# jannerm/ddpo

Hardware: AMD Instinct MI355X
Metric: sampled images/sec (512^2, 50 DDIM steps) (higher is better)
Workload: dtype f32 (f16mx: f16 MFMA + MX-fp8 cross terms on the long-reduction conv/GEMM layers, bf16x3-split MFMA elsewhere); 1 GPU; BASELINE configs[1]: compressed-animals geometry, sd15 U-Net+VAE (random init), 512x512, 50 DDIM steps, CFG 5.0, eta 1.0, sample_batch_size 8/GPU, VAE decode included; parallelism=dp1, global_batch=8

## Files before the change

ddpo_amd/csrc/attention_bf16.hip:

```cpp
#include "common.h"
#include <cstdlib>


typedef __bf16 bf16x8 __attribute__((ext_vector_type(8)));
typedef _Float16 f16x8 __attribute__((ext_vector_type(8)));
typedef _Float16 f16x2 __attribute__((ext_vector_type(2)));
typedef float f32x16 __attribute__((ext_vector_type(16)));

typedef __bf16 bf16x2 __attribute__((ext_vector_type(2)));
__device__ __forceinline__ uint32_t cvt_pk_bf16_a(float lo, float hi) {
  const bf16x2 v = {(__bf16)lo, (__bf16)hi};
  return __builtin_bit_cast(uint32_t, v);
}
__device__ __forceinline__ uint32_t cvt_pk_f16_a(float lo, float hi) {
  const f16x2 v = {(_Float16)lo, (_Float16)hi};
  return __builtin_bit_cast(uint32_t, v);
}
__device__ __forceinline__ void split2(float a, float b, uint32_t& hi, uint32_t& lo) {
  hi = cvt_pk_bf16_a(a, b);
  lo = cvt_pk_bf16_a(a - __uint_as_float(hi << 16), b - __uint_as_float(hi & 0xFFFF0000u));
}
__device__ __forceinline__ void split2h(float a, float b, uint32_t& hi, uint32_t& lo) {
  const float lim = 65504.f;
  a = fminf(fmaxf(a, -lim), lim);
  b = fminf(fmaxf(b, -lim), lim);
  hi = cvt_pk_f16_a(a, b);
  const f16x2 h = __builtin_bit_cast(f16x2, hi);
  lo = cvt_pk_f16_a(a - (float)h[0], b - (float)h[1]);
}
#define MFMA32(a, b, c) __builtin_amdgcn_mfma_f32_32x32x16_bf16((a), (b), (c), 0, 0, 0)
#define MFMA32H(a, b, c) __builtin_amdgcn_mfma_f32_32x32x16_f16((a), (b), (c), 0, 0, 0)
#define ATTN_P_SHIFT 14.0f
#define ATTN_F16_ONE 0x3C00u

template <bool ONES>
__device__ __forceinline__ void attn_softmax_tile(const f32x16 (&sacc)[2], float& m_run, float& l_run, f16x8 (&ph)[4], float& alpha, bool& grew) {
  float mx = sacc[0][0];
#pragma unroll
  for (int j = 0; j < 2; ++j)
#pragma unroll
    for (int r = 0; r < 16; ++r) mx = fmaxf(mx, sacc[j][r]);
  mx = fmaxf(mx, __shfl_xor(mx, 32, 64));
  const float m_new = fmaxf(m_run, mx);
  alpha = __builtin_amdgcn_exp2f(m_run - m_new);
  grew = m_new > m_run;
  m_run = m_new;
  const float m_sh = m_new - ATTN_P_SHIFT;
  float ls = 0.f;
#pragma unroll
  for (int j = 0; j < 2; ++j) {
#pragma unroll
    for (int half = 0; half < 2; ++half) {
      uint32_t pk[4];
#pragma unroll
      for (int e = 0; e < 4; ++e) {
        const float p0 = __builtin_amdgcn_exp2f(sacc[j][8 * half + 2 * e] - m_sh);
        const float p1 = __builtin_amdgcn_exp2f(sacc[j][8 * half + 2 * e + 1] - m_sh);
        pk[e] = cvt_pk_f16_a(p0, p1);
        if (!ONES) {
          const f16x2 q = __builtin_bit_cast(f16x2, pk[e]);
          ls += (float)q[0] + (float)q[1];
        }
      }
      ph[2 * j + half] = __builtin_bit_cast(f16x8, make_uint4(pk[0], pk[1], pk[2], pk[3]));
    }
  }
  if (!ONES) l_run = l_run * alpha + ls;
}

template <int NDT, int LDVT, int QB = 1>
__device__ __forceinline__ void attn_pv_tile(const char* Vhi, const char* Vlo, int li, int h, const f16x8 (*ph)[4], f32x16 (*oacc)[NDT]) {
  f16x8 vh[2][NDT], vl[2][NDT];
  auto fetch = [&](int u, int slot) {
#pragma unroll
    for (int n = 0; n < NDT; ++n) {
      const int off = ((32 * n + li) * LDVT + 16 * u + 4 * h) * 2;
      const uint2 a0 = *reinterpret_cast<const uint2*>(Vhi + off), a1 = *reinterpret_cast<const uint2*>(Vhi + off + 16);
      const uint2 c0 = *reinterpret_cast<const uint2*>(Vlo + off), c1 = *reinterpret_cast<const uint2*>(Vlo + off + 16);
      vh[slot][n] = __builtin_bit_cast(f16x8, make_uint4(a0.x, a0.y, a1.x, a1.y));
      vl[slot][n] = __builtin_bit_cast(f16x8, make_uint4(c0.x, c0.y, c1.x, c1.y));
    }
  };
  fetch(0, 0);
#pragma unroll
  for (int u = 0; u < 4; ++u) {
    if (u + 1 < 4) fetch(u + 1, (u + 1) & 1);
    __builtin_amdgcn_sched_barrier(0);
#pragma unroll
    for (int qb = 0; qb < QB; ++qb)
#pragma unroll
      for (int n = 0; n < NDT; ++n) oacc[qb][n] = MFMA32H(vl[u & 1][n], ph[qb][u], oacc[qb][n]);
#pragma unroll
    for (int qb = 0; qb < QB; ++qb)
#pragma unroll
      for (int n = 0; n < NDT; ++n) oacc[qb][n] = MFMA32H(vh[u & 1][n], ph[qb][u], oacc[qb][n]);
    __builtin_amdgcn_sched_barrier(0);
  }
}

template <int D, int NDT, bool ONES>
__device__ __forceinline__ float attn_row_sum(const f32x16 (&oacc)[NDT], float l_run, int li) {
  if constexpr (ONES) {
    constexpr int n1 = D / 32, r1 = D % 32;
    static_assert(r1 % 8 == 0 && n1 < NDT, "row D must be register 4 (r1 / 8) of the lanes with h == 0");
    return __shfl(oacc[n1][4 * (r1 / 8)], li, 64);
  } else {
    return l_run + __shfl_xor(l_run, 32, 64);
  }
}

__device__ __forceinline__ void attn_softmax_tile_x3(const f32x16 (&sacc)[2], float& m_run, float& l_run, bf16x8 (&ph)[4], bf16x8 (&pl)[4], float& alpha,
                                                     bool& grew) {
  float mx = sacc[0][0];
#pragma unroll
  for (int j = 0; j < 2; ++j)
#pragma unroll
    for (int r = 0; r < 16; ++r) mx = fmaxf(mx, sacc[j][r]);
  mx = fmaxf(mx, __shfl_xor(mx, 32, 64));
  const float m_new = fmaxf(m_run, mx);
  alpha = __builtin_amdgcn_exp2f(m_run - m_new);
  grew = m_new > m_run;
  m_run = m_new;
  float ls = 0.f;
#pragma unroll
  for (int j = 0; j < 2; ++j) {
#pragma unroll
    for (int half = 0; half < 2; ++half) {
      uint32_t hi[4], lo[4];
#pragma unroll
      for (int e = 0; e < 4; ++e) {
        const float p0 = __builtin_amdgcn_exp2f(sacc[j][8 * half + 2 * e] - m_new);
        const float p1 = __builtin_amdgcn_exp2f(sacc[j][8 * half + 2 * e + 1] - m_new);
        ls += p0 + p1;
        split2(p0, p1, hi[e], lo[e]);
      }
      ph[2 * j + half] = __builtin_bit_cast(bf16x8, make_uint4(hi[0], hi[1], hi[2], hi[3]));
      pl[2 * j + half] = __builtin_bit_cast(bf16x8, make_uint4(lo[0], lo[1], lo[2], lo[3]));
    }
  }
  l_run = l_run * alpha + ls;
}

template <int NDT, int LDVT, int QB = 1>
__device__ __forceinline__ void attn_pv_tile_x3(const char* Vhi, const char* Vlo, int li, int h, const bf16x8 (*ph)[4], const bf16x8 (*pl)[4],
                                                f32x16 (*oacc)[NDT]) {
#pragma unroll
  for (int u = 0; u < 4; ++u) {
#pragma unroll
    for (int n = 0; n < NDT; ++n) {
      const int off = ((32 * n + li) * LDVT + 16 * u + 4 * h) * 2;
      const uint2 a0 = *reinterpret_cast<const uint2*>(Vhi + off), a1 = *reinterpret_cast<const uint2*>(Vhi + off + 16);
      const uint2 c0 = *reinterpret_cast<const uint2*>(Vlo + off), c1 = *reinterpret_cast<const uint2*>(Vlo + off + 16);
      const bf16x8 vh = __builtin_bit_cast(bf16x8, make_uint4(a0.x, a0.y, a1.x, a1.y));
      const bf16x8 vl = __builtin_bit_cast(bf16x8, make_uint4(c0.x, c0.y, c1.x, c1.y));
#pragma unroll
      for (int qb = 0; qb < QB; ++qb) {
        oacc[qb][n] = MFMA32(vl, ph[qb][u], oacc[qb][n]);
        oacc[qb][n] = MFMA32(vh, pl[qb][u], oacc[qb][n]);
        oacc[qb][n] = MFMA32(vh, ph[qb][u], oacc[qb][n]);
      }
    }
  }
}

template <bool F16P, bool ONES, int NDT, int LDVT>
__device__ __forceinline__ void attn_tile_tail(const f32x16 (&sacc)[2], float& m_run, float& l_run, f32x16 (&oacc)[NDT], const char* Vhi, const char* Vlo,
                                               int li, int h) {
  float alpha;
  bool grew;
  if constexpr (F16P) {
    f16x8 ph[4];
    attn_softmax_tile<ONES>(sacc, m_run, l_run, ph, alpha, grew);
    if (__any(grew)) {
#pragma unroll
      for (int n = 0; n < NDT; ++n)
#pragma unroll
        for (int r = 0; r < 16; ++r) oacc[n][r] *= alpha;
    }
    attn_pv_tile<NDT, LDVT>(Vhi, Vlo, li, h, &ph, &oacc);
  } else {
    bf16x8 ph[4], pl[4];
    attn_softmax_tile_x3(sacc, m_run, l_run, ph, pl, alpha, grew);
    if (__any(grew)) {
#pragma unroll
      for (int n = 0; n < NDT; ++n)
#pragma unroll
        for (int r = 0; r < 16; ++r) oacc[n][r] *= alpha;
    }
    attn_pv_tile_x3<NDT, LDVT>(Vhi, Vlo, li, h, &ph, &pl, &oacc);
  }
}

struct AttnOut {
  float* o;
  uint16_t* hi;
  uint16_t* lo;
  int ld;
  int64_t rows;
};
template <int D, int NDT>
__device__ __forceinline__ void attn_store_o(const AttnOut out, int64_t row, int col0, const f32x16 (&oacc)[NDT], float inv, int h) {
#pragma unroll
  for (int n = 0; n < NDT; ++n) {
#pragma unroll
    for (int g = 0; g < 4; ++g) {
      const int dc = 32 * n + 8 * g + 4 * h;
      if (dc >= D) continue;
      const float v0 = oacc[n][4 * g] * inv, v1 = oacc[n][4 * g + 1] * inv, v2 = oacc[n][4 * g + 2] * inv, v3 = oacc[n][4 * g + 3] * inv;
      if (out.hi) {
        uint32_t h0, l0, h1, l1;
        split2(v0, v1, h0, l0);
        split2(v2, v3, h1, l1);
        const int64_t off = plane_off(row, col0 + dc, out.ld, out.rows);
        *reinterpret_cast<uint2*>(out.hi + off) = make_uint2(h0, h1);
        *reinterpret_cast<uint2*>(out.lo + off) = make_uint2(l0, l1);
      } else {
        *reinterpret_cast<float4*>(out.o + row * out.ld + col0 + dc) = make_float4(v0, v1, v2, v3);
      }
    }
  }
}


template <int D, int DKP, int DVP, bool F16P>
__global__ void __launch_bounds__(256) attn_fwd_bf16_kernel(const float* __restrict__ q, int ldq, const float* __restrict__ k, int ldk,
                                                            const float* __restrict__ v, int ldv, const AttnOut out,
                                                            float* __restrict__ lse, int heads, int Nq, int Nk, float scale_log2e, int qbat) {
  constexpr int KT = 64;
  constexpr int LDK = DKP + 8;
  constexpr int LDVT = KT + 4;
  constexpr int NKS = DKP / 16;
  constexpr int NDT = DVP / 32;
  constexpr bool ONES = F16P && DVP > D;
  constexpr int K_BYTES = KT * LDK * 2, VT_BYTES = DVP * LDVT * 2;
  __shared__ __attribute__((aligned(16))) char smem[2 * K_BYTES + 2 * VT_BYTES];
  char* Khi = smem; char* Klo = smem + K_BYTES;
  char* Vhi = smem + 2 * K_BYTES; char* Vlo = Vhi + VT_BYTES;

  const int t = threadIdx.x, lane = t & 63, wid = t >> 6;
  const int li = lane & 31, h = lane >> 5;
  const int bh = blockIdx.y, b = bh / heads, hd = bh - b * heads;
  const int q0 = blockIdx.x * 128 + wid * 32;
  const int qrow = min(q0 + li, Nq - 1);

  bf16x8 qh[NKS], ql[NKS];
  {
    const float* qp = q + ((int64_t)(b % qbat) * Nq + qrow) * ldq + hd * D;
#pragma unroll
    for (int s = 0; s < NKS; ++s) {
      uint32_t hi[4], lo[4];
#pragma unroll
      for (int e = 0; e < 4; ++e) {
        const int dk = 16 * s + 8 * h + 2 * e;
        const float a = dk < D ? qp[dk] * scale_log2e : 0.f;
        const float c = dk + 1 < D ? qp[dk + 1] * scale_log2e : 0.f;
        split2(a, c, hi[e], lo[e]);
      }
      qh[s] = __builtin_bit_cast(bf16x8, make_uint4(hi[0], hi[1], hi[2], hi[3]));
      ql[s] = __builtin_bit_cast(bf16x8, make_uint4(lo[0], lo[1], lo[2], lo[3]));
    }
  }
  for (int i = t; i < (2 * K_BYTES + 2 * VT_BYTES) / 16; i += 256) reinterpret_cast<uint4*>(smem)[i] = make_uint4(0u, 0u, 0u, 0u);
  if constexpr (ONES) {
    __syncthreads();
    if (t < KT) reinterpret_cast<uint16_t*>(Vhi)[D * LDVT + t] = (uint16_t)ATTN_F16_ONE;
  }

  f32x16 oacc[NDT];
#pragma unroll
  for (int n = 0; n < NDT; ++n)
#pragma unroll
    for (int r = 0; r < 16; ++r) oacc[n][r] = 0.f;
  float m_run = -INFINITY, l_run = 0.f;
  const float* kb = k + (int64_t)b * Nk * ldk + hd * D;
  const float* vb = v + (int64_t)b * Nk * ldv + hd * D;

  for (int kt0 = 0; kt0 < Nk; kt0 += KT) {
    __syncthreads();
    for (int i = t; i < KT * (D / 4); i += 256) {
      const int key = i / (D / 4), c4 = i - key * (D / 4);
      float4 kv = make_float4(0.f, 0.f, 0.f, 0.f), vv = kv;
      if (kt0 + key < Nk) {
        kv = *reinterpret_cast<const float4*>(kb + (int64_t)(kt0 + key) * ldk + c4 * 4);
        vv = *reinterpret_cast<const float4*>(vb + (int64_t)(kt0 + key) * ldv + c4 * 4);
      }
      uint32_t h0, l0, h1, l1;
      split2(kv.x, kv.y, h0, l0);
      split2(kv.z, kv.w, h1, l1);
      *reinterpret_cast<uint2*>(Khi + (key * LDK + c4 * 4) * 2) = make_uint2(h0, h1);
      *reinterpret_cast<uint2*>(Klo + (key * LDK + c4 * 4) * 2) = make_uint2(l0, l1);
      if (F16P) { split2h(vv.x, vv.y, h0, l0); split2h(vv.z, vv.w, h1, l1); }
      else { split2(vv.x, vv.y, h0, l0); split2(vv.z, vv.w, h1, l1); }
      uint16_t* vh = reinterpret_cast<uint16_t*>(Vhi);
      uint16_t* vl = reinterpret_cast<uint16_t*>(Vlo);
      const int d0 = c4 * 4;
      vh[(d0 + 0) * LDVT + key] = (uint16_t)(h0 & 0xFFFFu); vh[(d0 + 1) * LDVT + key] = (uint16_t)(h0 >> 16);
      vh[(d0 + 2) * LDVT + key] = (uint16_t)(h1 & 0xFFFFu); vh[(d0 + 3) * LDVT + key] = (uint16_t)(h1 >> 16);
      vl[(d0 + 0) * LDVT + key] = (uint16_t)(l0 & 0xFFFFu); vl[(d0 + 1) * LDVT + key] = (uint16_t)(l0 >> 16);
      vl[(d0 + 2) * LDVT + key] = (uint16_t)(l1 & 0xFFFFu); vl[(d0 + 3) * LDVT + key] = (uint16_t)(l1 >> 16);
    }
    __syncthreads();

    f32x16 sacc[2];
#pragma unroll
    for (int j = 0; j < 2; ++j)
#pragma unroll
      for (int r = 0; r < 16; ++r) sacc[j][r] = 0.f;
#pragma unroll
    for (int s = 0; s < NKS; ++s) {
#pragma unroll
      for (int j = 0; j < 2; ++j) {
        const int off = ((j * 32 + li) * LDK + 16 * s + 8 * h) * 2;
        const bf16x8 kh = *reinterpret_cast<const bf16x8*>(Khi + off);
        const bf16x8 kl = *reinterpret_cast<const bf16x8*>(Klo + off);
        sacc[j] = MFMA32(kl, qh[s], sacc[j]);
        sacc[j] = MFMA32(kh, ql[s], sacc[j]);
        sacc[j] = MFMA32(kh, qh[s], sacc[j]);
      }
    }
    if (kt0 + KT > Nk) {
#pragma unroll
      for (int j = 0; j < 2; ++j)
#pragma unroll
        for (int r = 0; r < 16; ++r)
          if (kt0 + 32 * j + (r & 3) + 8 * (r >> 2) + 4 * h >= Nk) sacc[j][r] = -INFINITY;
    }
    attn_tile_tail<F16P, ONES, NDT, LDVT>(sacc, m_run, l_run, oacc, Vhi, Vlo, li, h);
  }

  const float l_tot = attn_row_sum<D, NDT, ONES>(oacc, l_run, li);
  const float inv = 1.0f / l_tot;
  if (lse && h == 0 && q0 + li < Nq) lse[(int64_t)bh * Nq + q0 + li] = m_run + log2f(l_tot) - (F16P ? ATTN_P_SHIFT : 0.f);
  if (q0 + li < Nq) attn_store_o<D, NDT>(out, (int64_t)b * Nq + q0 + li, hd * D, oacc, inv, h);
}

template <int D, int DKP, int DVP>
struct AttnImg {
  static constexpr int KT = 64, LDK = DKP + 8, LDVT = KT + 4;
  static constexpr int K_BYTES = KT * LDK * 2, VT_BYTES = DVP * LDVT * 2;
  static constexpr int BYTES = 2 * K_BYTES + 2 * VT_BYTES;
  static constexpr int CHUNKS = BYTES / 16;
};

template <int D, int DKP, int DVP, bool F16P>
__global__ void __launch_bounds__(256) attn_pack_kv_kernel(const float* __restrict__ k, int ldk, const float* __restrict__ v, int ldv,
                                                           uint4* __restrict__ img, int heads, int Nk, int ntiles) {
  using I = AttnImg<D, DKP, DVP>;
  __shared__ __attribute__((aligned(16))) char smem[I::BYTES];
  char* Khi = smem; char* Klo = smem + I::K_BYTES;
  char* Vhi = smem + 2 * I::K_BYTES; char* Vlo = Vhi + I::VT_BYTES;
  const int t = threadIdx.x;
  const int tile = blockIdx.x, bh = blockIdx.y, b = bh / heads, hd = bh - b * heads;
  const int kt0 = tile * I::KT;
  for (int i = t; i < I::CHUNKS; i += 256) reinterpret_cast<uint4*>(smem)[i] = make_uint4(0u, 0u, 0u, 0u);
  __syncthreads();
  if (F16P && DVP > D && t < I::KT) reinterpret_cast<uint16_t*>(Vhi)[D * I::LDVT + t] = (uint16_t)ATTN_F16_ONE;
  const float* kb = k + (int64_t)b * Nk * ldk + hd * D;
  const float* vb = v + (int64_t)b * Nk * ldv + hd * D;
  for (int i = t; i < I::KT * (D / 4); i += 256) {
    const int key = i / (D / 4), c4 = i - key * (D / 4);
    if (kt0 + key >= Nk) continue;
    const float4 kv = *reinterpret_cast<const float4*>(kb + (int64_t)(kt0 + key) * ldk + c4 * 4);
    const float4 vv = *reinterpret_cast<const float4*>(vb + (int64_t)(kt0 + key) * ldv + c4 * 4);
    uint32_t h0, l0, h1, l1;
    split2(kv.x, kv.y, h0, l0);
    split2(kv.z, kv.w, h1, l1);
    *reinterpret_cast<uint2*>(Khi + (key * I::LDK + c4 * 4) * 2) = make_uint2(h0, h1);
    *reinterpret_cast<uint2*>(Klo + (key * I::LDK + c4 * 4) * 2) = make_uint2(l0, l1);
    if (F16P) { split2h(vv.x, vv.y, h0, l0); split2h(vv.z, vv.w, h1, l1); }
    else { split2(vv.x, vv.y, h0, l0); split2(vv.z, vv.w, h1, l1); }
    uint16_t* vh = reinterpret_cast<uint16_t*>(Vhi);
    uint16_t* vl = reinterpret_cast<uint16_t*>(Vlo);
    const int d0 = c4 * 4;
    vh[(d0 + 0) * I::LDVT + key] = (uint16_t)(h0 & 0xFFFFu); vh[(d0 + 1) * I::LDVT + key] = (uint16_t)(h0 >> 16);
    vh[(d0 + 2) * I::LDVT + key] = (uint16_t)(h1 & 0xFFFFu); vh[(d0 + 3) * I::LDVT + key] = (uint16_t)(h1 >> 16);
    vl[(d0 + 0) * I::LDVT + key] = (uint16_t)(l0 & 0xFFFFu); vl[(d0 + 1) * I::LDVT + key] = (uint16_t)(l0 >> 16);
    vl[(d0 + 2) * I::LDVT + key] = (uint16_t)(l1 & 0xFFFFu); vl[(d0 + 3) * I::LDVT + key] = (uint16_t)(l1 >> 16);
  }
  __syncthreads();
  uint4* dst = img + ((int64_t)bh * ntiles + tile) * I::CHUNKS;
  for (int i = t; i < I::CHUNKS; i += 256) dst[i] = reinterpret_cast<const uint4*>(smem)[i];
}

template <int D, int DKP, int DVP, bool F16P>
__global__ void __launch_bounds__(256, (DVP <= 32 ? 4 : (DKP <= 48 ? 3 : 2))) attn_fwd_bf16_pk_kernel(const float* __restrict__ q, int ldq, const uint4* __restrict__ img,
                                                               const AttnOut out, float* __restrict__ lse, int heads,
                                                               int Nq, int Nk, int ntiles, float scale_log2e, int qbat) {
  using I = AttnImg<D, DKP, DVP>;
  constexpr int KT = I::KT, LDK = I::LDK, LDVT = I::LDVT;
  constexpr int NKS = DKP / 16, NDT = DVP / 32;
  constexpr bool ONES = F16P && DVP > D;
  constexpr int NCH = (I::CHUNKS + 255) / 256;
  __shared__ __attribute__((aligned(16))) char smem[I::BYTES];
  const char* Khi = smem; const char* Klo = smem + I::K_BYTES;
  const char* Vhi = smem + 2 * I::K_BYTES; const char* Vlo = Vhi + I::VT_BYTES;

  const int t = threadIdx.x, lane = t & 63, wid = t >> 6;
  const int li = lane & 31, h = lane >> 5;
  const int bh = blockIdx.y, b = bh / heads, hd = bh - b * heads;
  const int q0 = blockIdx.x * 128 + wid * 32;
  const int qrow = min(q0 + li, Nq - 1);

  bf16x8 qh[NKS], ql[NKS];
  {
    const float* qp = q + ((int64_t)(b % qbat) * Nq + qrow) * ldq + hd * D;
#pragma unroll
    for (int s = 0; s < NKS; ++s) {
      uint32_t hi[4], lo[4];
#pragma unroll
      for (int e = 0; e < 4; ++e) {
        const int dk = 16 * s + 8 * h + 2 * e;
        const float a = dk < D ? qp[dk] * scale_log2e : 0.f;
        const float c = dk + 1 < D ? qp[dk + 1] * scale_log2e : 0.f;
        split2(a, c, hi[e], lo[e]);
      }
      qh[s] = __builtin_bit_cast(bf16x8, make_uint4(hi[0], hi[1], hi[2], hi[3]));
      ql[s] = __builtin_bit_cast(bf16x8, make_uint4(lo[0], lo[1], lo[2], lo[3]));
    }
  }

  f32x16 oacc[NDT];
#pragma unroll
  for (int n = 0; n < NDT; ++n)
#pragma unroll
    for (int r = 0; r < 16; ++r) oacc[n][r] = 0.f;
  float m_run = -INFINITY, l_run = 0.f;

  const uint4* src = img + (int64_t)bh * ntiles * I::CHUNKS;
  uint4 pre[NCH];
#pragma unroll
  for (int c = 0; c < NCH; ++c) {
    const int i = t + 256 * c;
    pre[c] = (NCH * 256 == I::CHUNKS || i < I::CHUNKS) ? src[i] : make_uint4(0u, 0u, 0u, 0u);
  }

  for (int tile = 0; tile < ntiles; ++tile) {
    const int kt0 = tile * KT;
    __syncthreads();
#pragma unroll
    for (int c = 0; c < NCH; ++c) {
      const int i = t + 256 * c;
      if (NCH * 256 == I::CHUNKS || i < I::CHUNKS) reinterpret_cast<uint4*>(smem)[i] = pre[c];
    }
    __syncthreads();
    {
      const uint4* nsrc = src + (int64_t)min(tile + 1, ntiles - 1) * I::CHUNKS;
#pragma unroll
      for (int c = 0; c < NCH; ++c) {
        const int i = t + 256 * c;
        pre[c] = (NCH * 256 == I::CHUNKS || i < I::CHUNKS) ? nsrc[i] : make_uint4(0u, 0u, 0u, 0u);
      }
    }

    f32x16 sacc[2];
#pragma unroll
    for (int j = 0; j < 2; ++j)
#pragma unroll
      for (int r = 0; r < 16; ++r) sacc[j][r] = 0.f;
#pragma unroll
    for (int s = 0; s < NKS; ++s) {
#pragma unroll
      for (int j = 0; j < 2; ++j) {
        const int off = ((j * 32 + li) * LDK + 16 * s + 8 * h) * 2;
        const bf16x8 kh = *reinterpret_cast<const bf16x8*>(Khi + off);
        const bf16x8 kl = *reinterpret_cast<const bf16x8*>(Klo + off);
        sacc[j] = MFMA32(kl, qh[s], sacc[j]);
        sacc[j] = MFMA32(kh, ql[s], sacc[j]);
        sacc[j] = MFMA32(kh, qh[s], sacc[j]);
      }
    }
    if (kt0 + KT > Nk) {
#pragma unroll
      for (int j = 0; j < 2; ++j)
#pragma unroll
        for (int r = 0; r < 16; ++r)
          if (kt0 + 32 * j + (r & 3) + 8 * (r >> 2) + 4 * h >= Nk) sacc[j][r] = -INFINITY;
    }
    attn_tile_tail<F16P, ONES, NDT, LDVT>(sacc, m_run, l_run, oacc, Vhi, Vlo, li, h);
  }

  const float l_tot = attn_row_sum<D, NDT, ONES>(oacc, l_run, li);
  const float inv = 1.0f / l_tot;
  if (lse && h == 0 && q0 + li < Nq) lse[(int64_t)bh * Nq + q0 + li] = m_run + log2f(l_tot) - (F16P ? ATTN_P_SHIFT : 0.f);
  if (q0 + li < Nq) attn_store_o<D, NDT>(out, (int64_t)b * Nq + q0 + li, hd * D, oacc, inv, h);
}

typedef unsigned int u32x4_a __attribute__((ext_vector_type(4)));

template <int D, int DKP, int DVP, int QB, bool F16P>
__global__ void __launch_bounds__(256, (QB == 2 ? 2 : (DVP <= 32 ? 4 : (DKP <= 48 ? 3 : 2)))) attn_fwd_bf16_dma_kernel(const float* __restrict__ q, int ldq, const uint4* __restrict__ img,
                                                               const AttnOut out, float* __restrict__ lse, int heads,
                                                               int Nq, int Nk, int ntiles, float scale_log2e, int qbat) {
  using I = AttnImg<D, DKP, DVP>;
  constexpr int KT = I::KT, LDK = I::LDK, LDVT = I::LDVT;
  constexpr int NKS = DKP / 16, NDT = DVP / 32;
  constexpr bool ONES = F16P && DVP > D;
  constexpr int KP = 2 * I::K_BYTES, VP = 2 * I::VT_BYTES;
  static_assert(KP % 1024 == 0 && VP % 1024 == 0, "LDS-DMA moves whole KiB pieces");
  constexpr int NPK = KP / 1024, NPV = VP / 1024;
  __shared__ __attribute__((aligned(1024))) char smem[2 * KP + VP];

  const int t = threadIdx.x, lane = t & 63, wid = t >> 6;
  const int wv = __builtin_amdgcn_readfirstlane(wid);
  const int li = lane & 31, h = lane >> 5;
  const int bh = blockIdx.y, b = bh / heads, hd = bh - b * heads;
  const int q0 = blockIdx.x * (128 * QB) + wid * (32 * QB);

  bf16x8 qh[QB][NKS], ql[QB][NKS];
#pragma unroll
  for (int qb = 0; qb < QB; ++qb) {
    const int qrow = min(q0 + 32 * qb + li, Nq - 1);
    const float* qp = q + ((int64_t)(b % qbat) * Nq + qrow) * ldq + hd * D;
#pragma unroll
    for (int s = 0; s < NKS; ++s) {
      uint32_t hi[4], lo[4];
#pragma unroll
      for (int e = 0; e < 4; ++e) {
        const int dk = 16 * s + 8 * h + 2 * e;
        const float a = dk < D ? qp[dk] * scale_log2e : 0.f;
        const float c = dk + 1 < D ? qp[dk + 1] * scale_log2e : 0.f;
        split2(a, c, hi[e], lo[e]);
      }
      qh[qb][s] = __builtin_bit_cast(bf16x8, make_uint4(hi[0], hi[1], hi[2], hi[3]));
      ql[qb][s] = __builtin_bit_cast(bf16x8, make_uint4(lo[0], lo[1], lo[2], lo[3]));
    }
  }

  f32x16 oacc[QB][NDT];
  float m_run[QB], l_run[QB];
#pragma unroll
  for (int qb = 0; qb < QB; ++qb) {
    m_run[qb] = -INFINITY; l_run[qb] = 0.f;
#pragma unroll
    for (int n = 0; n < NDT; ++n)
#pragma unroll
      for (int r = 0; r < 16; ++r) oacc[qb][n][r] = 0.f;
  }

  const uint64_t base = reinterpret_cast<uint64_t>(img + (int64_t)bh * ntiles * I::CHUNKS);
  const u32x4_a rs = {(uint32_t)base, (uint32_t)(base >> 32) & 0xFFFFu, 0x7FFFFFFFu, 0x00020000u};
  const uint32_t lds0 = (uint32_t)(uintptr_t)((__attribute__((address_space(3))) char*)smem);
  const uint32_t lane16 = (uint32_t)lane * 16u;
  auto fill = [&](uint32_t lds_region, uint32_t img_off, int npieces, int tile) {
    const uint32_t so = (uint32_t)tile * (uint32_t)I::BYTES + img_off;
    for (int p = wv; p < npieces; p += 4)
      asm volatile("s_nop 4\n\ts_mov_b32 m0, %0\n\ts_nop 0\n\tbuffer_load_dwordx4 %1, %2, %3 offen lds"
                   :: "s"(lds0 + lds_region + (uint32_t)p * 1024u), "v"(lane16 + (uint32_t)p * 1024u), "s"(rs), "s"(so) : "memory");
  };

  fill(0, 0, NPK, 0);
  for (int tile = 0; tile < ntiles; ++tile) {
    const int kt0 = tile * KT;
    const uint32_t kreg = (tile & 1) ? KP : 0;
    const char* Khi = smem + kreg; const char* Klo = Khi + I::K_BYTES;
    const char* Vhi = smem + 2 * KP; const char* Vlo = Vhi + I::VT_BYTES;
    asm volatile("s_waitcnt vmcnt(0) lgkmcnt(0)" ::: "memory");
    __builtin_amdgcn_s_barrier();
    fill(2 * KP, KP, NPV, tile);
    if (tile + 1 < ntiles) fill((tile & 1) ? 0 : KP, 0, NPK, tile + 1);

    f16x8 ph[QB][4];
    bf16x8 xh[QB][4], xl[QB][4];
#pragma unroll
    for (int qb = 0; qb < QB; ++qb) {
      f32x16 sacc[2];
  #pragma unroll
      for (int j = 0; j < 2; ++j)
  #pragma unroll
        for (int r = 0; r < 16; ++r) sacc[j][r] = 0.f;
  #pragma unroll
      for (int s = 0; s < NKS; ++s) {
  #pragma unroll
        for (int j = 0; j < 2; ++j) {
          const int off = ((j * 32 + li) * LDK + 16 * s + 8 * h) * 2;
          const bf16x8 kh = *reinterpret_cast<const bf16x8*>(Khi + off);
          const bf16x8 kl = *reinterpret_cast<const bf16x8*>(Klo + off);
          sacc[j] = MFMA32(kl, qh[qb][s], sacc[j]);
          sacc[j] = MFMA32(kh, ql[qb][s], sacc[j]);
          sacc[j] = MFMA32(kh, qh[qb][s], sacc[j]);
        }
      }
      if (kt0 + KT > Nk) {
  #pragma unroll
        for (int j = 0; j < 2; ++j)
  #pragma unroll
          for (int r = 0; r < 16; ++r)
            if (kt0 + 32 * j + (r & 3) + 8 * (r >> 2) + 4 * h >= Nk) sacc[j][r] = -INFINITY;
      }
      float alpha;
      bool grew;
      if constexpr (F16P) attn_softmax_tile<ONES>(sacc, m_run[qb], l_run[qb], ph[qb], alpha, grew);
      else attn_softmax_tile_x3(sacc, m_run[qb], l_run[qb], xh[qb], xl[qb], alpha, grew);
      if (__any(grew)) {
  #pragma unroll
        for (int n = 0; n < NDT; ++n)
  #pragma unroll
          for (int r = 0; r < 16; ++r) oacc[qb][n][r] *= alpha;
      }
    }
    asm volatile("s_waitcnt vmcnt(0) lgkmcnt(0)" ::: "memory");
    __builtin_amdgcn_s_barrier();
    if constexpr (F16P) attn_pv_tile<NDT, LDVT, QB>(Vhi, Vlo, li, h, ph, oacc);
    else attn_pv_tile_x3<NDT, LDVT, QB>(Vhi, Vlo, li, h, xh, xl, oacc);
  }

#pragma unroll
  for (int qb = 0; qb < QB; ++qb) {
    const int qi = q0 + 32 * qb + li;
    const float l_tot = attn_row_sum<D, NDT, ONES>(oacc[qb], l_run[qb], li);
    const float inv = 1.0f / l_tot;
    if (lse && h == 0 && qi < Nq) lse[(int64_t)bh * Nq + qi] = m_run[qb] + log2f(l_tot) - (F16P ? ATTN_P_SHIFT : 0.f);
    if (qi < Nq) attn_store_o<D, NDT>(out, (int64_t)b * Nq + qi, hd * D, oacc[qb], inv, h);
  }
}

#define ATTN_PK_MIN_NK 256

template <int D, int DKP, int DVP, bool F16P>
static int launch_pack_kv(const float* k, int ldk, const float* v, int ldv, uint4* img, int B, int heads, int Nk, hipStream_t st) {
  using I = AttnImg<D, DKP, DVP>;
  const int ntiles = (Nk + I::KT - 1) / I::KT;
  hipLaunchKernelGGL((attn_pack_kv_kernel<D, DKP, DVP, F16P>), dim3(ntiles, B * heads), dim3(256), 0, st, k, ldk, v, ldv, img, heads, Nk, ntiles);
  DDPO_LAUNCH_CHECK();
  return DDPO_OK;
}

template <int D, int DKP, int DVP, bool F16P>
static int launch_attn_images(const float* q, int ldq, int qbat, const uint4* img, const AttnOut& out, float* lse, int B, int heads, int Nq, int Nk,
                              float scale, hipStream_t st) {
  using I = AttnImg<D, DKP, DVP>;
  dim3 grid((Nq + 127) / 128, B * heads);
  const int ntiles = (Nk + I::KT - 1) / I::KT;
  if constexpr ((2 * I::K_BYTES) % 1024 == 0 && (2 * I::VT_BYTES) % 1024 == 0) {
    if ((int64_t)ntiles * I::BYTES < 0x7FFFFFFF) {
      hipLaunchKernelGGL((attn_fwd_bf16_dma_kernel<D, DKP, DVP, 1, F16P>), grid, dim3(256), 0, st, q, ldq, img, out, lse, heads, Nq, Nk, ntiles,
                         scale * 1.4426950408889634f, qbat);
      DDPO_LAUNCH_CHECK();
      return DDPO_OK;
    }
  }
  hipLaunchKernelGGL((attn_fwd_bf16_pk_kernel<D, DKP, DVP, F16P>), grid, dim3(256), 0, st, q, ldq, img, out, lse, heads, Nq, Nk, ntiles,
                     scale * 1.4426950408889634f, qbat);
  DDPO_LAUNCH_CHECK();
  return DDPO_OK;
}

template <int D, int DKP, int DVP, bool F16P>
static int launch_attn_bf16(const float* q, int ldq, int qbat, const float* k, int ldk, const float* v, int ldv, const AttnOut& out, float* lse,
                            int B, int heads, int Nq, int Nk, float scale, void* ws, size_t ws_bytes, hipStream_t st) {
  using I = AttnImg<D, DKP, DVP>;
  dim3 grid((Nq + 127) / 128, B * heads);
  const int ntiles = (Nk + I::KT - 1) / I::KT;
  const size_t need = (size_t)B * heads * ntiles * I::BYTES;
  if (Nk >= ATTN_PK_MIN_NK && ws && ws_bytes >= need && !(reinterpret_cast<uintptr_t>(ws) & 15)) {
    uint4* img = reinterpret_cast<uint4*>(ws);
    const int rc = launch_pack_kv<D, DKP, DVP, F16P>(k, ldk, v, ldv, img, B, heads, Nk, st);
    if (rc != DDPO_OK) return rc;
    return launch_attn_images<D, DKP, DVP, F16P>(q, ldq, qbat, img, out, lse, B, heads, Nq, Nk, scale, st);
  }
  hipLaunchKernelGGL((attn_fwd_bf16_kernel<D, DKP, DVP, F16P>), grid, dim3(256), 0, st, q, ldq, k, ldk, v, ldv, out, lse, heads, Nq, Nk,
                     scale * 1.4426950408889634f, qbat);
  DDPO_LAUNCH_CHECK();
  return DDPO_OK;
}

template <int D, int DKP, int DVP>
static size_t attn_img_bytes(int B, int heads, int Nk) {
  using I = AttnImg<D, DKP, DVP>;
  return (size_t)B * heads * ((Nk + I::KT - 1) / I::KT) * I::BYTES;
}
template <int D, int DKP, int DVP>
static size_t attn_ws(int B, int heads, int Nk) {
  if (Nk < ATTN_PK_MIN_NK) return 0;
  return attn_img_bytes<D, DKP, DVP>(B, heads, Nk);
}

extern "C" size_t ddpo_attention_fwd_bf16x3_ws_bytes(int B, int heads, int Nk, int d) {
  if (B <= 0 || heads <= 0 || Nk <= 0) return 0;
  switch (d) {
    case 8:  return attn_ws<8, 16, 32>(B, heads, Nk);
    case 16: return attn_ws<16, 16, 32>(B, heads, Nk);
    case 40: return attn_ws<40, 48, 64>(B, heads, Nk);
    case 64: return attn_ws<64, 64, 64>(B, heads, Nk);
    case 80: return attn_ws<80, 80, 96>(B, heads, Nk);
    default: return 0;
  }
}

#define ATTN_BY_D(CALL)                                      \
  switch (d) {                                               \
    case 8:  return CALL(8, 16, 32);                         \
    case 16: return CALL(16, 16, 32);                        \
    case 40: return CALL(40, 48, 64);                        \
    case 64: return CALL(64, 64, 64);                        \
    case 80: return CALL(80, 80, 96);                        \
    default: return DDPO_EINVAL;  \
  }

static bool attn_out_ok(const AttnOut& out, int heads, int d) {
  if (out.hi) {
    if (!out.lo || out.o || (out.ld & 3) || ((reinterpret_cast<uintptr_t>(out.hi) | reinterpret_cast<uintptr_t>(out.lo)) & 7)) return false;
    return out.ld != 0 || ((heads * d) & 31) == 0;
  }
  return out.o && !(out.ld & 3) && !(reinterpret_cast<uintptr_t>(out.o) & 15);
}

template <bool F16P>
static int attention_fwd_impl(const float* q, int ldq, int qbat, const float* k, int ldk, const float* v, int ldv, const AttnOut& out,
                              float* lse, int B, int heads, int Nq, int Nk, int d, float scale, void* ws, size_t ws_bytes, void* stream) {
  if (!q || !k || !v || B <= 0 || heads <= 0 || Nq <= 0 || Nk <= 0 || d <= 0 || !attn_out_ok(out, heads, d)) return DDPO_EINVAL;
  if ((ldq & 3) || (ldk & 3) || (ldv & 3) || (long)B * heads > 65535) return DDPO_EINVAL;
  if ((reinterpret_cast<uintptr_t>(q) | reinterpret_cast<uintptr_t>(k) | reinterpret_cast<uintptr_t>(v)) & 15) return DDPO_EINVAL;
  if (qbat < 1 || qbat > B || B % qbat) return DDPO_EINVAL;
  hipStream_t st = as_stream(stream);
#define CALL(DD, DK, DV) launch_attn_bf16<DD, DK, DV, F16P>(q, ldq, qbat, k, ldk, v, ldv, out, lse, B, heads, Nq, Nk, scale, ws, ws_bytes, st)
  ATTN_BY_D(CALL)
#undef CALL
}
extern "C" int ddpo_attention_fwd_bf16x3(const float* q, int ldq, const float* k, int ldk, const float* v, int ldv, float* o, int ldo,
                                         float* lse, int B, int heads, int Nq, int Nk, int d, float scale, void* ws, size_t ws_bytes,
                                         void* stream) {
  return attention_fwd_impl<false>(q, ldq, B, k, ldk, v, ldv, AttnOut{o, nullptr, nullptr, ldo, (int64_t)B * Nq}, lse, B, heads, Nq, Nk, d, scale, ws,
                                   ws_bytes, stream);
}
extern "C" int ddpo_attention_fwd_f16p(const float* q, int ldq, const float* k, int ldk, const float* v, int ldv, float* o, int ldo,
                                       float* lse, int B, int heads, int Nq, int Nk, int d, float scale, void* ws, size_t ws_bytes,
                                       void* stream) {
  return attention_fwd_impl<true>(q, ldq, B, k, ldk, v, ldv, AttnOut{o, nullptr, nullptr, ldo, (int64_t)B * Nq}, lse, B, heads, Nq, Nk, d, scale, ws,
                                  ws_bytes, stream);
}
extern "C" int ddpo_attention_fwd_bf16x3_po(const float* q, int ldq, const float* k, int ldk, const float* v, int ldv, uint16_t* o_hi,
                                            uint16_t* o_lo, int ld_planes, float* lse, int B, int heads, int Nq, int Nk, int d, float scale,
                                            void* ws, size_t ws_bytes, void* stream) {
  if (!o_hi) return DDPO_EINVAL;
  return attention_fwd_impl<false>(q, ldq, B, k, ldk, v, ldv, AttnOut{nullptr, o_hi, o_lo, ld_planes, (int64_t)B * Nq}, lse, B, heads, Nq, Nk, d, scale,
                                   ws, ws_bytes, stream);
}
extern "C" int ddpo_attention_fwd_f16p_po(const float* q, int ldq, const float* k, int ldk, const float* v, int ldv, uint16_t* o_hi,
                                          uint16_t* o_lo, int ld_planes, float* lse, int B, int heads, int Nq, int Nk, int d, float scale,
                                          void* ws, size_t ws_bytes, void* stream) {
  if (!o_hi) return DDPO_EINVAL;
  return attention_fwd_impl<true>(q, ldq, B, k, ldk, v, ldv, AttnOut{nullptr, o_hi, o_lo, ld_planes, (int64_t)B * Nq}, lse, B, heads, Nq, Nk, d, scale,
                                  ws, ws_bytes, stream);
}

extern "C" size_t ddpo_attention_kv_images_bytes(int B, int heads, int Nk, int d) {
  if (B <= 0 || heads <= 0 || Nk <= 0) return 0;
  switch (d) {
    case 8:  return attn_img_bytes<8, 16, 32>(B, heads, Nk);
    case 16: return attn_img_bytes<16, 16, 32>(B, heads, Nk);
    case 40: return attn_img_bytes<40, 48, 64>(B, heads, Nk);
    case 64: return attn_img_bytes<64, 64, 64>(B, heads, Nk);
    case 80: return attn_img_bytes<80, 80, 96>(B, heads, Nk);
    default: return 0;
  }
}

template <bool F16P>
static int pack_kv_impl(const float* k, int ldk, const float* v, int ldv, void* images, size_t images_bytes, int B, int heads, int Nk, int d,
                        void* stream) {
  if (!k || !v || !images || B <= 0 || heads <= 0 || Nk <= 0 || (ldk & 3) || (ldv & 3) || (long)B * heads > 65535) return DDPO_EINVAL;
  if ((reinterpret_cast<uintptr_t>(k) | reinterpret_cast<uintptr_t>(v) | reinterpret_cast<uintptr_t>(images)) & 15) return DDPO_EINVAL;
  const size_t need = ddpo_attention_kv_images_bytes(B, heads, Nk, d);
  if (need == 0 || images_bytes < need) return DDPO_EINVAL;
  hipStream_t st = as_stream(stream);
  uint4* img = reinterpret_cast<uint4*>(images);
#define CALL(DD, DK, DV) launch_pack_kv<DD, DK, DV, F16P>(k, ldk, v, ldv, img, B, heads, Nk, st)
  ATTN_BY_D(CALL)
#undef CALL
}
extern "C" int ddpo_attention_pack_kv_bf16x3(const float* k, int ldk, const float* v, int ldv, void* images, size_t images_bytes, int B, int heads,
                                             int Nk, int d, void* stream) {
  return pack_kv_impl<false>(k, ldk, v, ldv, images, images_bytes, B, heads, Nk, d, stream);
}
extern "C" int ddpo_attention_pack_kv_f16p(const float* k, int ldk, const float* v, int ldv, void* images, size_t images_bytes, int B, int heads,
                                           int Nk, int d, void* stream) {
  return pack_kv_impl<true>(k, ldk, v, ldv, images, images_bytes, B, heads, Nk, d, stream);
}

template <bool F16P>
static int attention_images_impl(const float* q, int ldq, int qbat, const void* images, size_t images_bytes, const AttnOut& out, float* lse,
                                 int B, int heads, int Nq, int Nk, int d, float scale, void* stream) {
  if (!q || !images || B <= 0 || heads <= 0 || Nq <= 0 || Nk <= 0 || d <= 0 || !attn_out_ok(out, heads, d)) return DDPO_EINVAL;
  if ((ldq & 3) || (long)B * heads > 65535) return DDPO_EINVAL;
  if (qbat < 1 || qbat > B || B % qbat) return DDPO_EINVAL;
  if ((reinterpret_cast<uintptr_t>(q) | reinterpret_cast<uintptr_t>(images)) & 15) return DDPO_EINVAL;
  const size_t need = ddpo_attention_kv_images_bytes(B, heads, Nk, d);
  if (need == 0 || images_bytes < need) return DDPO_EINVAL;
  hipStream_t st = as_stream(stream);
  const uint4* img = reinterpret_cast<const uint4*>(images);
#define CALL(DD, DK, DV) launch_attn_images<DD, DK, DV, F16P>(q, ldq, qbat, img, out, lse, B, heads, Nq, Nk, scale, st)
  ATTN_BY_D(CALL)
#undef CALL
}
extern "C" int ddpo_attention_fwd_bf16x3_images(const float* q, int ldq, const void* images, size_t images_bytes, float* o, int ldo, float* lse,
                                                int B, int heads, int Nq, int Nk, int d, float scale, void* stream) {
  return attention_images_impl<false>(q, ldq, B, images, images_bytes, AttnOut{o, nullptr, nullptr, ldo, (int64_t)B * Nq}, lse, B, heads, Nq, Nk, d,
                                      scale, stream);
}
extern "C" int ddpo_attention_fwd_f16p_images(const float* q, int ldq, const void* images, size_t images_bytes, float* o, int ldo, float* lse,
                                              int B, int heads, int Nq, int Nk, int d, float scale, void* stream) {
  return attention_images_impl<true>(q, ldq, B, images, images_bytes, AttnOut{o, nullptr, nullptr, ldo, (int64_t)B * Nq}, lse, B, heads, Nq, Nk, d,
                                     scale, stream);
}
extern "C" int ddpo_attention_fwd_bf16x3_images_po(const float* q, int ldq, const void* images, size_t images_bytes, uint16_t* o_hi, uint16_t* o_lo,
                                                   int ld_planes, float* lse, int B, int heads, int Nq, int Nk, int d, float scale, void* stream) {
  if (!o_hi) return DDPO_EINVAL;
  return attention_images_impl<false>(q, ldq, B, images, images_bytes, AttnOut{nullptr, o_hi, o_lo, ld_planes, (int64_t)B * Nq}, lse, B, heads, Nq, Nk,
                                      d, scale, stream);
}
extern "C" int ddpo_attention_fwd_f16p_images_po(const float* q, int ldq, const void* images, size_t images_bytes, uint16_t* o_hi, uint16_t* o_lo,
                                                 int ld_planes, float* lse, int B, int heads, int Nq, int Nk, int d, float scale, void* stream) {
  if (!o_hi) return DDPO_EINVAL;
  return attention_images_impl<true>(q, ldq, B, images, images_bytes, AttnOut{nullptr, o_hi, o_lo, ld_planes, (int64_t)B * Nq}, lse, B, heads, Nq, Nk,
                                     d, scale, stream);
}

static bool shared_q_out(float* o, int ldo, uint16_t* o_hi, uint16_t* o_lo, int ld_planes, int64_t rows, AttnOut& out) {
  if (o_hi) {
    if (o) return false;
    out = AttnOut{nullptr, o_hi, o_lo, ld_planes, rows};
  } else {
    out = AttnOut{o, nullptr, nullptr, ldo, rows};
  }
  return true;
}
extern "C" int ddpo_attention_fwd_x16_shared_q(int f16p, const float* q, int ldq, int q_batches, const float* k, int ldk, const float* v, int ldv,
                                               float* o, int ldo, uint16_t* o_hi, uint16_t* o_lo, int ld_planes, float* lse, int B, int heads,
                                               int Nq, int Nk, int d, float scale, void* ws, size_t ws_bytes, void* stream) {
  AttnOut out;
  if (!shared_q_out(o, ldo, o_hi, o_lo, ld_planes, (int64_t)B * Nq, out)) return DDPO_EINVAL;
  return f16p ? attention_fwd_impl<true>(q, ldq, q_batches, k, ldk, v, ldv, out, lse, B, heads, Nq, Nk, d, scale, ws, ws_bytes, stream)
              : attention_fwd_impl<false>(q, ldq, q_batches, k, ldk, v, ldv, out, lse, B, heads, Nq, Nk, d, scale, ws, ws_bytes, stream);
}
extern "C" int ddpo_attention_fwd_images_shared_q(int f16p, const float* q, int ldq, int q_batches, const void* images, size_t images_bytes,
                                                  float* o, int ldo, uint16_t* o_hi, uint16_t* o_lo, int ld_planes, float* lse, int B, int heads,
                                                  int Nq, int Nk, int d, float scale, void* stream) {
  AttnOut out;
  if (!shared_q_out(o, ldo, o_hi, o_lo, ld_planes, (int64_t)B * Nq, out)) return DDPO_EINVAL;
  return f16p ? attention_images_impl<true>(q, ldq, q_batches, images, images_bytes, out, lse, B, heads, Nq, Nk, d, scale, stream)
              : attention_images_impl<false>(q, ldq, q_batches, images, images_bytes, out, lse, B, heads, Nq, Nk, d, scale, stream);
}
```

Before: 4.382 images/sec.

## Stack hi/lo K and V halves into shared tiles for head dim 40 attention

For head dimension 40, the key image now packs the bf16 hi and lo halves side by side in one padded 80-wide row. The V image also stacks its f16 lo rows below the hi rows in a 96-row tile, so a single MFMA pass covers both halves. This is meant to cut the MFMA count and LDS footprint of the bf16x3 score product and the f16 PV product, removing the padding waste from 40→48/64. Partial sums for the lo rows are folded back into the output at store time. The change adds a permuted Q fragment layout and an env toggle (DDPO_ATTN_STACK, on by default), and raises the occupancy hint to 3.

After: 4.447 images/sec, median of 6. +1.5%, better.

```diff
diff --git a/ddpo_amd/csrc/attention_bf16.hip b/ddpo_amd/csrc/attention_bf16.hip
--- a/ddpo_amd/csrc/attention_bf16.hip
+++ b/ddpo_amd/csrc/attention_bf16.hip
@@ -32,6 +32,143 @@
 #define MFMA32H(a, b, c) __builtin_amdgcn_mfma_f32_32x32x16_f16((a), (b), (c), 0, 0, 0)
 #define ATTN_P_SHIFT 14.0f
 #define ATTN_F16_ONE 0x3C00u
+
+constexpr bool attn_kstk(int D, int DKP) { return D == 40 && DKP == 2 * D; }
+template <int D, int DKP, int DVP>
+struct AttnImg {
+  static constexpr int KT = 64, LDK = DKP + 8, LDVT = KT + 4;
+  static constexpr bool KSTK = attn_kstk(D, DKP), VSTK = KSTK && DVP / 2 > D;
+  static constexpr int K_BYTES = KT * LDK * 2, VT_BYTES = DVP * LDVT * 2;
+  static constexpr int KP = KSTK ? K_BYTES : 2 * K_BYTES;
+  static constexpr int VP = VSTK ? (VT_BYTES + 1023) / 1024 * 1024 : 2 * VT_BYTES;
+  static constexpr int KLO = KSTK ? D * 2 : K_BYTES;
+  static constexpr int VLO = VSTK ? (DVP / 2) * LDVT * 2 : VT_BYTES;
+  static constexpr int NDT = DVP / 32;
+  static constexpr int BYTES = KP + VP;
+  static constexpr int CHUNKS = BYTES / 16;
+};
+
+template <class I, int D, bool ONES>
+__device__ __forceinline__ void attn_image_init(char* smem, int t) {
+  for (int i = t; i < I::CHUNKS; i += 256) reinterpret_cast<uint4*>(smem)[i] = make_uint4(0u, 0u, 0u, 0u);
+  if constexpr (ONES) {
+    __syncthreads();
+    if (t < I::KT) reinterpret_cast<uint16_t*>(smem + I::KP)[D * I::LDVT + t] = (uint16_t)ATTN_F16_ONE;
+  }
+}
+
+template <class I, int D, bool F16P>
+__device__ __forceinline__ void attn_stage_tile(char* smem, const float* kb, int ldk, const float* vb, int ldv, int kt0, int Nk, int t) {
+  char* Khi = smem; char* Klo = Khi + I::KLO;
+  uint16_t* vh = reinterpret_cast<uint16_t*>(smem + I::KP);
+  uint16_t* vl = reinterpret_cast<uint16_t*>(smem + I::KP + I::VLO);
+  for (int i = t; i < I::KT * (D / 4); i += 256) {
+    const int key = i / (D / 4), c4 = i - key * (D / 4);
+    float4 kv = make_float4(0.f, 0.f, 0.f, 0.f), vv = kv;
+    if (kt0 + key < Nk) {
+      kv = *reinterpret_cast<const float4*>(kb + (int64_t)(kt0 + key) * ldk + c4 * 4);
+      vv = *reinterpret_cast<const float4*>(vb + (int64_t)(kt0 + key) * ldv + c4 * 4);
+    }
+    uint32_t h0, l0, h1, l1;
+    split2(kv.x, kv.y, h0, l0);
+    split2(kv.z, kv.w, h1, l1);
+    *reinterpret_cast<uint2*>(Khi + (key * I::LDK + c4 * 4) * 2) = make_uint2(h0, h1);
+    *reinterpret_cast<uint2*>(Klo + (key * I::LDK + c4 * 4) * 2) = make_uint2(l0, l1);
+    if (F16P) { split2h(vv.x, vv.y, h0, l0); split2h(vv.z, vv.w, h1, l1); }
+    else { split2(vv.x, vv.y, h0, l0); split2(vv.z, vv.w, h1, l1); }
+    const int d0 = c4 * 4;
+    vh[(d0 + 0) * I::LDVT + key] = (uint16_t)(h0 & 0xFFFFu); vh[(d0 + 1) * I::LDVT + key] = (uint16_t)(h0 >> 16);
+    vh[(d0 + 2) * I::LDVT + key] = (uint16_t)(h1 & 0xFFFFu); vh[(d0 + 3) * I::LDVT + key] = (uint16_t)(h1 >> 16);
+    vl[(d0 + 0) * I::LDVT + key] = (uint16_t)(l0 & 0xFFFFu); vl[(d0 + 1) * I::LDVT + key] = (uint16_t)(l0 >> 16);
+    vl[(d0 + 2) * I::LDVT + key] = (uint16_t)(l1 & 0xFFFFu); vl[(d0 + 3) * I::LDVT + key] = (uint16_t)(l1 >> 16);
+  }
+}
+
+template <int D, int DKP>
+struct AttnQFrag {
+  static constexpr bool STK = attn_kstk(D, DKP);
+  static constexpr int N = STK ? 8 : 2 * (DKP / 16);
+  bf16x8 f[N];
+  __device__ __forceinline__ void load(const float* qp, float scale_log2e, int h) {
+    if constexpr (STK) {
+      uint4 qh[5], ql[5];
+#pragma unroll
+      for (int c = 0; c < 5; ++c) {
+        const float4 a = reinterpret_cast<const float4*>(qp)[2 * c], b = reinterpret_cast<const float4*>(qp)[2 * c + 1];
+        split2(a.x * scale_log2e, a.y * scale_log2e, qh[c].x, ql[c].x);
+        split2(a.z * scale_log2e, a.w * scale_log2e, qh[c].y, ql[c].y);
+        split2(b.x * scale_log2e, b.y * scale_log2e, qh[c].z, ql[c].z);
+        split2(b.z * scale_log2e, b.w * scale_log2e, qh[c].w, ql[c].w);
+      }
+      auto sel = [&](const uint4& a1, const uint4& a0) {
+        return __builtin_bit_cast(bf16x8, make_uint4(h ? a1.x : a0.x, h ? a1.y : a0.y, h ? a1.z : a0.z, h ? a1.w : a0.w));
+      };
+      const uint4 zero = make_uint4(0u, 0u, 0u, 0u);
+      f[0] = sel(qh[1], qh[0]); f[1] = sel(qh[3], qh[2]); f[2] = sel(qh[0], qh[4]); f[3] = sel(qh[2], qh[1]); f[4] = sel(qh[4], qh[3]);
+      f[5] = sel(ql[1], ql[0]); f[6] = sel(ql[3], ql[2]); f[7] = sel(zero, ql[4]);
+    } else {
+#pragma unroll
+      for (int s = 0; s < DKP / 16; ++s) {
+        uint32_t hi[4], lo[4];
+#pragma unroll
+        for (int e = 0; e < 4; ++e) {
+          const int dk = 16 * s + 8 * h + 2 * e;
+          const float a = dk < D ? qp[dk] * scale_log2e : 0.f;
+          const float c = dk + 1 < D ? qp[dk + 1] * scale_log2e : 0.f;
+          split2(a, c, hi[e], lo[e]);
+        }
+        f[2 * s] = __builtin_bit_cast(bf16x8, make_uint4(hi[0], hi[1], hi[2], hi[3]));
+        f[2 * s + 1] = __builtin_bit_cast(bf16x8, make_uint4(lo[0], lo[1], lo[2], lo[3]));
+      }
+    }
+  }
+};
+
+template <int D, int DKP, int DVP>
+__device__ __forceinline__ void attn_scores_tile(const char* K, int li, int h, const AttnQFrag<D, DKP>& q, f32x16 (&sacc)[2]) {
+  using I = AttnImg<D, DKP, DVP>;
+#pragma unroll
+  for (int j = 0; j < 2; ++j)
+#pragma unroll
+    for (int r = 0; r < 16; ++r) sacc[j][r] = 0.f;
+  if constexpr (I::KSTK) {
+    const int off7 = h ? 160 : 64;
+#pragma unroll
+    for (int i = 0; i < 8; ++i) {
+      const int s = i < 5 ? i + 3 : (i == 5 ? 2 : i - 6);
+#pragma unroll
+      for (int j = 0; j < 2; ++j) {
+        const int row = (j * 32 + li) * I::LDK * 2;
+        const int off = s < 5 ? 32 * s + 16 * h : (s < 7 ? 32 * (s - 5) + 16 * h : off7);
+        sacc[j] = MFMA32(*reinterpret_cast<const bf16x8*>(K + row + off), q.f[s], sacc[j]);
+      }
+    }
+  } else {
+    const char* Khi = K; const char* Klo = K + I::KLO;
+#pragma unroll
+    for (int s = 0; s < DKP / 16; ++s) {
+#pragma unroll
+      for (int j = 0; j < 2; ++j) {
+        const int off = ((j * 32 + li) * I::LDK + 16 * s + 8 * h) * 2;
+        const bf16x8 kh = *reinterpret_cast<const bf16x8*>(Khi + off);
+        const bf16x8 kl = *reinterpret_cast<const bf16x8*>(Klo + off);
+        sacc[j] = MFMA32(kl, q.f[2 * s], sacc[j]);
+        sacc[j] = MFMA32(kh, q.f[2 * s + 1], sacc[j]);
+        sacc[j] = MFMA32(kh, q.f[2 * s], sacc[j]);
+      }
+    }
+  }
+}
+
+__device__ __forceinline__ void attn_mask_tail(f32x16 (&sacc)[2], int kt0, int Nk, int h) {
+  if (kt0 + 64 > Nk) {
+#pragma unroll
+    for (int j = 0; j < 2; ++j)
+#pragma unroll
+      for (int r = 0; r < 16; ++r)
+        if (kt0 + 32 * j + (r & 3) + 8 * (r >> 2) + 4 * h >= Nk) sacc[j][r] = -INFINITY;
+  }
+}
 
 template <bool ONES>
 __device__ __forceinline__ void attn_softmax_tile(const f32x16 (&sacc)[2], float& m_run, float& l_run, f16x8 (&ph)[4], float& alpha, bool& grew) {
@@ -68,17 +205,19 @@
   if (!ONES) l_run = l_run * alpha + ls;
 }
 
-template <int NDT, int LDVT, int QB = 1>
+template <int NDT, int LDVT, int QB = 1, bool VSTK = false>
 __device__ __forceinline__ void attn_pv_tile(const char* Vhi, const char* Vlo, int li, int h, const f16x8 (*ph)[4], f32x16 (*oacc)[NDT]) {
-  f16x8 vh[2][NDT], vl[2][NDT];
+  f16x8 vh[2][NDT], vl[2][VSTK ? 1 : NDT];
   auto fetch = [&](int u, int slot) {
 #pragma unroll
     for (int n = 0; n < NDT; ++n) {
       const int off = ((32 * n + li) * LDVT + 16 * u + 4 * h) * 2;
       const uint2 a0 = *reinterpret_cast<const uint2*>(Vhi + off), a1 = *reinterpret_cast<const uint2*>(Vhi + off + 16);
-      const uint2 c0 = *reinterpret_cast<const uint2*>(Vlo + off), c1 = *reinterpret_cast<const uint2*>(Vlo + off + 16);
       vh[slot][n] = __builtin_bit_cast(f16x8, make_uint4(a0.x, a0.y, a1.x, a1.y));
-      vl[slot][n] = __builtin_bit_cast(f16x8, make_uint4(c0.x, c0.y, c1.x, c1.y));
+      if constexpr (!VSTK) {
+        const uint2 c0 = *reinterpret_cast<const uint2*>(Vlo + off), c1 = *reinterpret_cast<const uint2*>(Vlo + off + 16);
+        vl[slot][n] = __builtin_bit_cast(f16x8, make_uint4(c0.x, c0.y, c1.x, c1.y));
+      }
     }
   };
   fetch(0, 0);
@@ -86,10 +225,12 @@
   for (int u = 0; u < 4; ++u) {
     if (u + 1 < 4) fetch(u + 1, (u + 1) & 1);
     __builtin_amdgcn_sched_barrier(0);
-#pragma unroll
-    for (int qb = 0; qb < QB; ++qb)
-#pragma unroll
-      for (int n = 0; n < NDT; ++n) oacc[qb][n] = MFMA32H(vl[u & 1][n], ph[qb][u], oacc[qb][n]);
+    if constexpr (!VSTK) {
+#pragma unroll
+      for (int qb = 0; qb < QB; ++qb)
+#pragma unroll
+        for (int n = 0; n < NDT; ++n) oacc[qb][n] = MFMA32H(vl[u & 1][n], ph[qb][u], oacc[qb][n]);
+    }
 #pragma unroll
     for (int qb = 0; qb < QB; ++qb)
 #pragma unroll
@@ -163,7 +304,7 @@
   }
 }
 
-template <bool F16P, bool ONES, int NDT, int LDVT>
+template <bool F16P, bool ONES, int NDT, int LDVT, bool VSTK>
 __device__ __forceinline__ void attn_tile_tail(const f32x16 (&sacc)[2], float& m_run, float& l_run, f32x16 (&oacc)[NDT], const char* Vhi, const char* Vlo,
                                                int li, int h) {
   float alpha;
@@ -177,7 +318,7 @@
 #pragma unroll
         for (int r = 0; r < 16; ++r) oacc[n][r] *= alpha;
     }
-    attn_pv_tile<NDT, LDVT>(Vhi, Vlo, li, h, &ph, &oacc);
+    attn_pv_tile<NDT, LDVT, 1, VSTK>(Vhi, Vlo, li, h, &ph, &oacc);
   } else {
     bf16x8 ph[4], pl[4];
     attn_softmax_tile_x3(sacc, m_run, l_run, ph, pl, alpha, grew);
@@ -198,15 +339,22 @@
   int ld;
   int64_t rows;
 };
-template <int D, int NDT>
+template <int D, int NDT, bool VSTK = false>
 __device__ __forceinline__ void attn_store_o(const AttnOut out, int64_t row, int col0, const f32x16 (&oacc)[NDT], float inv, int h) {
+  static_assert(!VSTK || (NDT == 3 && D % 8 == 0), "lo rows at +48 = one tile and two register groups further");
 #pragma unroll
   for (int n = 0; n < NDT; ++n) {
 #pragma unroll
     for (int g = 0; g < 4; ++g) {
       const int dc = 32 * n + 8 * g + 4 * h;
       if (dc >= D) continue;
-      const float v0 = oacc[n][4 * g] * inv, v1 = oacc[n][4 * g + 1] * inv, v2 = oacc[n][4 * g + 2] * inv, v3 = oacc[n][4 * g + 3] * inv;
+      float v0 = oacc[n][4 * g], v1 = oacc[n][4 * g + 1], v2 = oacc[n][4 * g + 2], v3 = oacc[n][4 * g + 3];
+      if constexpr (VSTK) {
+        if (32 * n + 8 * g >= D) continue;
+        const int n2 = g < 2 ? n + 1 : n + 2, g2 = g < 2 ? g + 2 : g - 2;
+        v0 += oacc[n2][4 * g2]; v1 += oacc[n2][4 * g2 + 1]; v2 += oacc[n2][4 * g2 + 2]; v3 += oacc[n2][4 * g2 + 3];
+      }
+      v0 *= inv; v1 *= inv; v2 *= inv; v3 *= inv;
       if (out.hi) {
         uint32_t h0, l0, h1, l1;
         split2(v0, v1, h0, l0);
@@ -223,19 +371,14 @@
 
 
 template <int D, int DKP, int DVP, bool F16P>
-__global__ void __launch_bounds__(256) attn_fwd_bf16_kernel(const float* __restrict__ q, int ldq, const float* __restrict__ k, int ldk,
+__global__ void __launch_bounds__(256, (attn_kstk(D, DKP) ? 3 : 1)) attn_fwd_bf16_kernel(const float* __restrict__ q, int ldq, const float* __restrict__ k, int ldk,
                                                             const float* __restrict__ v, int ldv, const AttnOut out,
                                                             float* __restrict__ lse, int heads, int Nq, int Nk, float scale_log2e, int qbat) {
-  constexpr int KT = 64;
-  constexpr int LDK = DKP + 8;
-  constexpr int LDVT = KT + 4;
-  constexpr int NKS = DKP / 16;
-  constexpr int NDT = DVP / 32;
+  using I = AttnImg<D, DKP, DVP>;
+  constexpr int KT = I::KT, LDVT = I::LDVT, NDT = I::NDT;
   constexpr bool ONES = F16P && DVP > D;
-  constexpr int K_BYTES = KT * LDK * 2, VT_BYTES = DVP * LDVT * 2;
-  __shared__ __attribute__((aligned(16))) char smem[2 * K_BYTES + 2 * VT_BYTES];
-  char* Khi = smem; char* Klo = smem + K_BYTES;
-  char* Vhi = smem + 2 * K_BYTES; char* Vlo = Vhi + VT_BYTES;
+  __shared__ __attribute__((aligned(16))) char smem[I::BYTES];
+  const char* Vhi = smem + I::KP; const char* Vlo = Vhi + I::VLO;
 
   const int t = threadIdx.x, lane = t & 63, wid = t >> 6;
   const int li = lane & 31, h = lane >> 5;
@@ -243,28 +386,9 @@
   const int q0 = blockIdx.x * 128 + wid * 32;
   const int qrow = min(q0 + li, Nq - 1);
 
-  bf16x8 qh[NKS], ql[NKS];
-  {
-    const float* qp = q + ((int64_t)(b % qbat) * Nq + qrow) * ldq + hd * D;
-#pragma unroll
-    for (int s = 0; s < NKS; ++s) {
-      uint32_t hi[4], lo[4];
-#pragma unroll
-      for (int e = 0; e < 4; ++e) {
-        const int dk = 16 * s + 8 * h + 2 * e;
-        const float a = dk < D ? qp[dk] * scale_log2e : 0.f;
-        const float c = dk + 1 < D ? qp[dk + 1] * scale_log2e : 0.f;
-        split2(a, c, hi[e], lo[e]);
-      }
-      qh[s] = __builtin_bit_cast(bf16x8, make_uint4(hi[0], hi[1], hi[2], hi[3]));
-      ql[s] = __builtin_bit_cast(bf16x8, make_uint4(lo[0], lo[1], lo[2], lo[3]));
-    }
-  }
-  for (int i = t; i < (2 * K_BYTES + 2 * VT_BYTES) / 16; i += 256) reinterpret_cast<uint4*>(smem)[i] = make_uint4(0u, 0u, 0u, 0u);
-  if constexpr (ONES) {
-    __syncthreads();
-    if (t < KT) reinterpret_cast<uint16_t*>(Vhi)[D * LDVT + t] = (uint16_t)ATTN_F16_ONE;
-  }
+  AttnQFrag<D, DKP> qf;
+  qf.load(q + ((int64_t)(b % qbat) * Nq + qrow) * ldq + hd * D, scale_log2e, h);
+  attn_image_init<I, D, ONES>(smem, t);
 
   f32x16 oacc[NDT];
 #pragma unroll
@@ -277,123 +401,45 @@
 
   for (int kt0 = 0; kt0 < Nk; kt0 += KT) {
     __syncthreads();
-    for (int i = t; i < KT * (D / 4); i += 256) {
-      const int key = i / (D / 4), c4 = i - key * (D / 4);
-      float4 kv = make_float4(0.f, 0.f, 0.f, 0.f), vv = kv;
-      if (kt0 + key < Nk) {
-        kv = *reinterpret_cast<const float4*>(kb + (int64_t)(kt0 + key) * ldk + c4 * 4);
-        vv = *reinterpret_cast<const float4*>(vb + (int64_t)(kt0 + key) * ldv + c4 * 4);
-      }
-      uint32_t h0, l0, h1, l1;
-      split2(kv.x, kv.y, h0, l0);
-      split2(kv.z, kv.w, h1, l1);
-      *reinterpret_cast<uint2*>(Khi + (key * LDK + c4 * 4) * 2) = make_uint2(h0, h1);
-      *reinterpret_cast<uint2*>(Klo + (key * LDK + c4 * 4) * 2) = make_uint2(l0, l1);
-      if (F16P) { split2h(vv.x, vv.y, h0, l0); split2h(vv.z, vv.w, h1, l1); }
-      else { split2(vv.x, vv.y, h0, l0); split2(vv.z, vv.w, h1, l1); }
-      uint16_t* vh = reinterpret_cast<uint16_t*>(Vhi);
-      uint16_t* vl = reinterpret_cast<uint16_t*>(Vlo);
-      const int d0 = c4 * 4;
-      vh[(d0 + 0) * LDVT + key] = (uint16_t)(h0 & 0xFFFFu); vh[(d0 + 1) * LDVT + key] = (uint16_t)(h0 >> 16);
-      vh[(d0 + 2) * LDVT + key] = (uint16_t)(h1 & 0xFFFFu); vh[(d0 + 3) * LDVT + key] = (uint16_t)(h1 >> 16);
-      vl[(d0 + 0) * LDVT + key] = (uint16_t)(l0 & 0xFFFFu); vl[(d0 + 1) * LDVT + key] = (uint16_t)(l0 >> 16);
-      vl[(d0 + 2) * LDVT + key] = (uint16_t)(l1 & 0xFFFFu); vl[(d0 + 3) * LDVT + key] = (uint16_t)(l1 >> 16);
-    }
+    attn_stage_tile<I, D, F16P>(smem, kb, ldk, vb, ldv, kt0, Nk, t);
     __syncthreads();
-
     f32x16 sacc[2];
-#pragma unroll
-    for (int j = 0; j < 2; ++j)
-#pragma unroll
-      for (int r = 0; r < 16; ++r) sacc[j][r] = 0.f;
-#pragma unroll
-    for (int s = 0; s < NKS; ++s) {
-#pragma unroll
-      for (int j = 0; j < 2; ++j) {
-        const int off = ((j * 32 + li) * LDK + 16 * s + 8 * h) * 2;
-        const bf16x8 kh = *reinterpret_cast<const bf16x8*>(Khi + off);
-        const bf16x8 kl = *reinterpret_cast<const bf16x8*>(Klo + off);
-        sacc[j] = MFMA32(kl, qh[s], sacc[j]);
-        sacc[j] = MFMA32(kh, ql[s], sacc[j]);
-        sacc[j] = MFMA32(kh, qh[s], sacc[j]);
-      }
-    }
-    if (kt0 + KT > Nk) {
-#pragma unroll
-      for (int j = 0; j < 2; ++j)
-#pragma unroll
-        for (int r = 0; r < 16; ++r)
-          if (kt0 + 32 * j + (r & 3) + 8 * (r >> 2) + 4 * h >= Nk) sacc[j][r] = -INFINITY;
-    }
-    attn_tile_tail<F16P, ONES, NDT, LDVT>(sacc, m_run, l_run, oacc, Vhi, Vlo, li, h);
+    attn_scores_tile<D, DKP, DVP>(smem, li, h, qf, sacc);
+    attn_mask_tail(sacc, kt0, Nk, h);
+    attn_tile_tail<F16P, ONES, NDT, LDVT, I::VSTK>(sacc, m_run, l_run, oacc, Vhi, Vlo, li, h);
   }
 
   const float l_tot = attn_row_sum<D, NDT, ONES>(oacc, l_run, li);
   const float inv = 1.0f / l_tot;
   if (lse && h == 0 && q0 + li < Nq) lse[(int64_t)bh * Nq + q0 + li] = m_run + log2f(l_tot) - (F16P ? ATTN_P_SHIFT : 0.f);
-  if (q0 + li < Nq) attn_store_o<D, NDT>(out, (int64_t)b * Nq + q0 + li, hd * D, oacc, inv, h);
-}
-
-template <int D, int DKP, int DVP>
-struct AttnImg {
-  static constexpr int KT = 64, LDK = DKP + 8, LDVT = KT + 4;
-  static constexpr int K_BYTES = KT * LDK * 2, VT_BYTES = DVP * LDVT * 2;
-  static constexpr int BYTES = 2 * K_BYTES + 2 * VT_BYTES;
-  static constexpr int CHUNKS = BYTES / 16;
-};
+  if (q0 + li < Nq) attn_store_o<D, NDT, I::VSTK>(out, (int64_t)b * Nq + q0 + li, hd * D, oacc, inv, h);
+}
 
 template <int D, int DKP, int DVP, bool F16P>
 __global__ void __launch_bounds__(256) attn_pack_kv_kernel(const float* __restrict__ k, int ldk, const float* __restrict__ v, int ldv,
                                                            uint4* __restrict__ img, int heads, int Nk, int ntiles) {
   using I = AttnImg<D, DKP, DVP>;
   __shared__ __attribute__((aligned(16))) char smem[I::BYTES];
-  char* Khi = smem; char* Klo = smem + I::K_BYTES;
-  char* Vhi = smem + 2 * I::K_BYTES; char* Vlo = Vhi + I::VT_BYTES;
   const int t = threadIdx.x;
   const int tile = blockIdx.x, bh = blockIdx.y, b = bh / heads, hd = bh - b * heads;
-  const int kt0 = tile * I::KT;
-  for (int i = t; i < I::CHUNKS; i += 256) reinterpret_cast<uint4*>(smem)[i] = make_uint4(0u, 0u, 0u, 0u);
+  attn_image_init<I, D, (F16P && DVP > D)>(smem, t);
   __syncthreads();
-  if (F16P && DVP > D && t < I::KT) reinterpret_cast<uint16_t*>(Vhi)[D * I::LDVT + t] = (uint16_t)ATTN_F16_ONE;
-  const float* kb = k + (int64_t)b * Nk * ldk + hd * D;
-  const float* vb = v + (int64_t)b * Nk * ldv + hd * D;
-  for (int i = t; i < I::KT * (D / 4); i += 256) {
-    const int key = i / (D / 4), c4 = i - key * (D / 4);
-    if (kt0 + key >= Nk) continue;
-    const float4 kv = *reinterpret_cast<const float4*>(kb + (int64_t)(kt0 + key) * ldk + c4 * 4);
-    const float4 vv = *reinterpret_cast<const float4*>(vb + (int64_t)(kt0 + key) * ldv + c4 * 4);
-    uint32_t h0, l0, h1, l1;
-    split2(kv.x, kv.y, h0, l0);
-    split2(kv.z, kv.w, h1, l1);
-    *reinterpret_cast<uint2*>(Khi + (key * I::LDK + c4 * 4) * 2) = make_uint2(h0, h1);
-    *reinterpret_cast<uint2*>(Klo + (key * I::LDK + c4 * 4) * 2) = make_uint2(l0, l1);
-    if (F16P) { split2h(vv.x, vv.y, h0, l0); split2h(vv.z, vv.w, h1, l1); }
-    else { split2(vv.x, vv.y, h0, l0); split2(vv.z, vv.w, h1, l1); }
-    uint16_t* vh = reinterpret_cast<uint16_t*>(Vhi);
-    uint16_t* vl = reinterpret_cast<uint16_t*>(Vlo);
-    const int d0 = c4 * 4;
-    vh[(d0 + 0) * I::LDVT + key] = (uint16_t)(h0 & 0xFFFFu); vh[(d0 + 1) * I::LDVT + key] = (uint16_t)(h0 >> 16);
-    vh[(d0 + 2) * I::LDVT + key] = (uint16_t)(h1 & 0xFFFFu); vh[(d0 + 3) * I::LDVT + key] = (uint16_t)(h1 >> 16);
-    vl[(d0 + 0) * I::LDVT + key] = (uint16_t)(l0 & 0xFFFFu); vl[(d0 + 1) * I::LDVT + key] = (uint16_t)(l0 >> 16);
-    vl[(d0 + 2) * I::LDVT + key] = (uint16_t)(l1 & 0xFFFFu); vl[(d0 + 3) * I::LDVT + key] = (uint16_t)(l1 >> 16);
-  }
+  attn_stage_tile<I, D, F16P>(smem, k + (int64_t)b * Nk * ldk + hd * D, ldk, v + (int64_t)b * Nk * ldv + hd * D, ldv, tile * I::KT, Nk, t);
   __syncthreads();
   uint4* dst = img + ((int64_t)bh * ntiles + tile) * I::CHUNKS;
   for (int i = t; i < I::CHUNKS; i += 256) dst[i] = reinterpret_cast<const uint4*>(smem)[i];
 }
 
 template <int D, int DKP, int DVP, bool F16P>
-__global__ void __launch_bounds__(256, (DVP <= 32 ? 4 : (DKP <= 48 ? 3 : 2))) attn_fwd_bf16_pk_kernel(const float* __restrict__ q, int ldq, const uint4* __restrict__ img,
+__global__ void __launch_bounds__(256, (DVP <= 32 ? 4 : (DKP <= 48 || attn_kstk(D, DKP) ? 3 : 2))) attn_fwd_bf16_pk_kernel(const float* __restrict__ q, int ldq, const uint4* __restrict__ img,
                                                                const AttnOut out, float* __restrict__ lse, int heads,
                                                                int Nq, int Nk, int ntiles, float scale_log2e, int qbat) {
   using I = AttnImg<D, DKP, DVP>;
-  constexpr int KT = I::KT, LDK = I::LDK, LDVT = I::LDVT;
-  constexpr int NKS = DKP / 16, NDT = DVP / 32;
+  constexpr int KT = I::KT, LDVT = I::LDVT, NDT = I::NDT;
   constexpr bool ONES = F16P && DVP > D;
   constexpr int NCH = (I::CHUNKS + 255) / 256;
   __shared__ __attribute__((aligned(16))) char smem[I::BYTES];
-  const char* Khi = smem; const char* Klo = smem + I::K_BYTES;
-  const char* Vhi = smem + 2 * I::K_BYTES; const char* Vlo = Vhi + I::VT_BYTES;
+  const char* Vhi = smem + I::KP; const char* Vlo = Vhi + I::VLO;
 
   const int t = threadIdx.x, lane = t & 63, wid = t >> 6;
   const int li = lane & 31, h = lane >> 5;
@@ -401,23 +447,8 @@
   const int q0 = blockIdx.x * 128 + wid * 32;
   const int qrow = min(q0 + li, Nq - 1);
 
-  bf16x8 qh[NKS], ql[NKS];
-  {
-    const float* qp = q + ((int64_t)(b % qbat) * Nq + qrow) * ldq + hd * D;
-#pragma unroll
-    for (int s = 0; s < NKS; ++s) {
-      uint32_t hi[4], lo[4];
-#pragma unroll
-      for (int e = 0; e < 4; ++e) {
-        const int dk = 16 * s + 8 * h + 2 * e;
-        const float a = dk < D ? qp[dk] * scale_log2e : 0.f;
-        const float c = dk + 1 < D ? qp[dk + 1] * scale_log2e : 0.f;
-        split2(a, c, hi[e], lo[e]);
-      }
-      qh[s] = __builtin_bit_cast(bf16x8, make_uint4(hi[0], hi[1], hi[2], hi[3]));
-      ql[s] = __builtin_bit_cast(bf16x8, make_uint4(lo[0], lo[1], lo[2], lo[3]));
-    }
-  }
+  AttnQFrag<D, DKP> qf;
+  qf.load(q + ((int64_t)(b % qbat) * Nq + qrow) * ldq + hd * D, scale_log2e, h);
 
   f32x16 oacc[NDT];
 #pragma unroll
@@ -453,49 +484,27 @@
     }
 
     f32x16 sacc[2];
-#pragma unroll
-    for (int j = 0; j < 2; ++j)
-#pragma unroll
-      for (int r = 0; r < 16; ++r) sacc[j][r] = 0.f;
-#pragma unroll
-    for (int s = 0; s < NKS; ++s) {
-#pragma unroll
-      for (int j = 0; j < 2; ++j) {
-        const int off = ((j * 32 + li) * LDK + 16 * s + 8 * h) * 2;
-        const bf16x8 kh = *reinterpret_cast<const bf16x8*>(Khi + off);
-        const bf16x8 kl = *reinterpret_cast<const bf16x8*>(Klo + off);
-        sacc[j] = MFMA32(kl, qh[s], sacc[j]);
-        sacc[j] = MFMA32(kh, ql[s], sacc[j]);
-        sacc[j] = MFMA32(kh, qh[s], sacc[j]);
-      }
-    }
-    if (kt0 + KT > Nk) {
-#pragma unroll
-      for (int j = 0; j < 2; ++j)
-#pragma unroll
-        for (int r = 0; r < 16; ++r)
-          if (kt0 + 32 * j + (r & 3) + 8 * (r >> 2) + 4 * h >= Nk) sacc[j][r] = -INFINITY;
-    }
-    attn_tile_tail<F16P, ONES, NDT, LDVT>(sacc, m_run, l_run, oacc, Vhi, Vlo, li, h);
+    attn_scores_tile<D, DKP, DVP>(smem, li, h, qf, sacc);
+    attn_mask_tail(sacc, kt0, Nk, h);
+    attn_tile_tail<F16P, ONES, NDT, LDVT, I::VSTK>(sacc, m_run, l_run, oacc, Vhi, Vlo, li, h);
   }
 
   const float l_tot = attn_row_sum<D, NDT, ONES>(oacc, l_run, li);
   const float inv = 1.0f / l_tot;
   if (lse && h == 0 && q0 + li < Nq) lse[(int64_t)bh * Nq + q0 + li] = m_run + log2f(l_tot) - (F16P ? ATTN_P_SHIFT : 0.f);
-  if (q0 + li < Nq) attn_store_o<D, NDT>(out, (int64_t)b * Nq + q0 + li, hd * D, oacc, inv, h);
+  if (q0 + li < Nq) attn_store_o<D, NDT, I::VSTK>(out, (int64_t)b * Nq + q0 + li, hd * D, oacc, inv, h);
 }
 
 typedef unsigned int u32x4_a __attribute__((ext_vector_type(4)));
 
 template <int D, int DKP, int DVP, int QB, bool F16P>
-__global__ void __launch_bounds__(256, (QB == 2 ? 2 : (DVP <= 32 ? 4 : (DKP <= 48 ? 3 : 2)))) attn_fwd_bf16_dma_kernel(const float* __restrict__ q, int ldq, const uint4* __restrict__ img,
+__global__ void __launch_bounds__(256, (QB == 2 ? 2 : (DVP <= 32 ? 4 : (DKP <= 48 || attn_kstk(D, DKP) ? 3 : 2)))) attn_fwd_bf16_dma_kernel(const float* __restrict__ q, int ldq, const uint4* __restrict__ img,
                                                                const AttnOut out, float* __restrict__ lse, int heads,
                                                                int Nq, int Nk, int ntiles, float scale_log2e, int qbat) {
   using I = AttnImg<D, DKP, DVP>;
-  constexpr int KT = I::KT, LDK = I::LDK, LDVT = I::LDVT;
-  constexpr int NKS = DKP / 16, NDT = DVP / 32;
+  constexpr int KT = I::KT, LDVT = I::LDVT, NDT = I::NDT;
   constexpr bool ONES = F16P && DVP > D;
-  constexpr int KP = 2 * I::K_BYTES, VP = 2 * I::VT_BYTES;
+  constexpr int KP = I::KP, VP = I::VP;
   static_assert(KP % 1024 == 0 && VP % 1024 == 0, "LDS-DMA moves whole KiB pieces");
   constexpr int NPK = KP / 1024, NPV = VP / 1024;
   __shared__ __attribute__((aligned(1024))) char smem[2 * KP + VP];
@@ -506,24 +515,11 @@
   const int bh = blockIdx.y, b = bh / heads, hd = bh - b * heads;
   const int q0 = blockIdx.x * (128 * QB) + wid * (32 * QB);
 
-  bf16x8 qh[QB][NKS], ql[QB][NKS];
+  AttnQFrag<D, DKP> qf[QB];
 #pragma unroll
   for (int qb = 0; qb < QB; ++qb) {
     const int qrow = min(q0 + 32 * qb + li, Nq - 1);
-    const float* qp = q + ((int64_t)(b % qbat) * Nq + qrow) * ldq + hd * D;
-#pragma unroll
-    for (int s = 0; s < NKS; ++s) {
-      uint32_t hi[4], lo[4];
-#pragma unroll
-      for (int e = 0; e < 4; ++e) {
-        const int dk = 16 * s + 8 * h + 2 * e;
-        const float a = dk < D ? qp[dk] * scale_log2e : 0.f;
-        const float c = dk + 1 < D ? qp[dk + 1] * scale_log2e : 0.f;
-        split2(a, c, hi[e], lo[e]);
-      }
-      qh[qb][s] = __builtin_bit_cast(bf16x8, make_uint4(hi[0], hi[1], hi[2], hi[3]));
-      ql[qb][s] = __builtin_bit_cast(bf16x8, make_uint4(lo[0], lo[1], lo[2], lo[3]));
-    }
+    qf[qb].load(q + ((int64_t)(b % qbat) * Nq + qrow) * ldq + hd * D, scale_log2e, h);
   }
 
   f32x16 oacc[QB][NDT];
@@ -552,8 +548,7 @@
   for (int tile = 0; tile < ntiles; ++tile) {
     const int kt0 = tile * KT;
     const uint32_t kreg = (tile & 1) ? KP : 0;
-    const char* Khi = smem + kreg; const char* Klo = Khi + I::K_BYTES;
-    const char* Vhi = smem + 2 * KP; const char* Vlo = Vhi + I::VT_BYTES;
+    const char* Vhi = smem + 2 * KP; const char* Vlo = Vhi + I::VLO;
     asm volatile("s_waitcnt vmcnt(0) lgkmcnt(0)" ::: "memory");
     __builtin_amdgcn_s_barrier();
     fill(2 * KP, KP, NPV, tile);
@@ -564,29 +559,8 @@
 #pragma unroll
     for (int qb = 0; qb < QB; ++qb) {
       f32x16 sacc[2];
-  #pragma unroll
-      for (int j = 0; j < 2; ++j)
-  #pragma unroll
-        for (int r = 0; r < 16; ++r) sacc[j][r] = 0.f;
-  #pragma unroll
-      for (int s = 0; s < NKS; ++s) {
-  #pragma unroll
-        for (int j = 0; j < 2; ++j) {
-          const int off = ((j * 32 + li) * LDK + 16 * s + 8 * h) * 2;
-          const bf16x8 kh = *reinterpret_cast<const bf16x8*>(Khi + off);
-          const bf16x8 kl = *reinterpret_cast<const bf16x8*>(Klo + off);
-          sacc[j] = MFMA32(kl, qh[qb][s], sacc[j]);
-          sacc[j] = MFMA32(kh, ql[qb][s], sacc[j]);
-          sacc[j] = MFMA32(kh, qh[qb][s], sacc[j]);
-        }
-      }
-      if (kt0 + KT > Nk) {
-  #pragma unroll
-        for (int j = 0; j < 2; ++j)
-  #pragma unroll
-          for (int r = 0; r < 16; ++r)
-            if (kt0 + 32 * j + (r & 3) + 8 * (r >> 2) + 4 * h >= Nk) sacc[j][r] = -INFINITY;
-      }
+      attn_scores_tile<D, DKP, DVP>(smem + kreg, li, h, qf[qb], sacc);
+      attn_mask_tail(sacc, kt0, Nk, h);
       float alpha;
       bool grew;
       if constexpr (F16P) attn_softmax_tile<ONES>(sacc, m_run[qb], l_run[qb], ph[qb], alpha, grew);
@@ -600,7 +574,7 @@
     }
     asm volatile("s_waitcnt vmcnt(0) lgkmcnt(0)" ::: "memory");
     __builtin_amdgcn_s_barrier();
-    if constexpr (F16P) attn_pv_tile<NDT, LDVT, QB>(Vhi, Vlo, li, h, ph, oacc);
+    if constexpr (F16P) attn_pv_tile<NDT, LDVT, QB, I::VSTK>(Vhi, Vlo, li, h, ph, oacc);
     else attn_pv_tile_x3<NDT, LDVT, QB>(Vhi, Vlo, li, h, xh, xl, oacc);
   }
 
@@ -610,7 +584,7 @@
     const float l_tot = attn_row_sum<D, NDT, ONES>(oacc[qb], l_run[qb], li);
     const float inv = 1.0f / l_tot;
     if (lse && h == 0 && qi < Nq) lse[(int64_t)bh * Nq + qi] = m_run[qb] + log2f(l_tot) - (F16P ? ATTN_P_SHIFT : 0.f);
-    if (qi < Nq) attn_store_o<D, NDT>(out, (int64_t)b * Nq + qi, hd * D, oacc[qb], inv, h);
+    if (qi < Nq) attn_store_o<D, NDT, I::VSTK>(out, (int64_t)b * Nq + qi, hd * D, oacc[qb], inv, h);
   }
 }
 
@@ -631,7 +605,7 @@
   using I = AttnImg<D, DKP, DVP>;
   dim3 grid((Nq + 127) / 128, B * heads);
   const int ntiles = (Nk + I::KT - 1) / I::KT;
-  if constexpr ((2 * I::K_BYTES) % 1024 == 0 && (2 * I::VT_BYTES) % 1024 == 0) {
+  if constexpr (I::KP % 1024 == 0 && I::VP % 1024 == 0) {
     if ((int64_t)ntiles * I::BYTES < 0x7FFFFFFF) {
       hipLaunchKernelGGL((attn_fwd_bf16_dma_kernel<D, DKP, DVP, 1, F16P>), grid, dim3(256), 0, st, q, ldq, img, out, lse, heads, Nq, Nk, ntiles,
                          scale * 1.4426950408889634f, qbat);
@@ -687,11 +661,19 @@
   }
 }
 
+static bool attn_stack() {
+  static const bool on = [] {
+    const char* e = getenv("DDPO_ATTN_STACK");
+    return !(e && e[0] == '0');
+  }();
+  return on;
+}
+
 #define ATTN_BY_D(CALL)                                      \
   switch (d) {                                               \
     case 8:  return CALL(8, 16, 32);                         \
     case 16: return CALL(16, 16, 32);                        \
-    case 40: return CALL(40, 48, 64);                        \
+    case 40: return attn_stack() ? CALL(40, 80, (F16P ? 96 : 64)) : CALL(40, 48, 64);  \
     case 64: return CALL(64, 64, 64);                        \
     case 80: return CALL(80, 80, 96);                        \
     default: return DDPO_EINVAL;  \
```
